# lucidrains/ring-attention-pytorch

Measured on AMD Instinct MI355X. Metric: attn_tflops, higher is better.
Workload: dtype bf16; 1 GPU; model=ring_flash_attn (non-causal, d_head 64), global_batch=1, seq_len=8192, seq_per_gpu=8192, heads=8, kv_heads=8, d_head=64, parallelism=ring1, hipgraph=True

## Files before the change

ring_attention_amd/csrc/attn_fwd.hip:

```cpp

#include <hip/hip_runtime.h>
#include <hip/hip_bf16.h>
#include <cstdint>
#include <cstdlib>

#include "attn_common.h"

namespace ring_attn {

static constexpr int WAVES = 8;
static constexpr int QROWS_WAVE = 32;
static constexpr int QROWS_WG = ROWS_WG;
static_assert(QROWS_WG == WAVES * QROWS_WAVE);
static constexpr int NTHREADS = WAVES * 64;

template <int D>
struct FwdLds {
    static constexpr int KVB = kvblk(D);
    __align__(16) __bf16 k[2][KVB * D];
    __align__(16) __bf16 vt[2][D * KVB];
    unsigned char kmask[2][KVB];
};

template <int D, bool SOFTCLAMP, bool PAIRED>
__global__ __launch_bounds__(NTHREADS, 1) void attn_fwd_kernel(FwdParams p) {
    static_assert(D % 32 == 0);
    constexpr int DBLK = D / 32;
    constexpr int KSTEPS = D / 16;
    constexpr int KVBLK = kvblk(D);
    constexpr int NBLK = KVBLK / 32;

    __shared__ FwdLds<D> lds;

    const int tid = threadIdx.x;
    const int lane = tid & 63;
    const int wid = tid >> 6;
    const int l31 = lane & 31;
    const int lhi = lane >> 5;

    const int bh = blockIdx.y;
    const int b = bh / p.h;
    const int h = bh % p.h;
    const int hk = h % p.hk;

    const int n_pit = PAIRED
        ? (p.paired - 1 - (int)blockIdx.x == (int)blockIdx.x ? 1 : 2) : 1;
    for (int pit = 0; pit < n_pit; ++pit) {
    const int qtile = PAIRED
        ? (pit == 0 ? (int)blockIdx.x : p.paired - 1 - (int)blockIdx.x)
        : (int)blockIdx.x;
    if (PAIRED && pit == 1) {
        __syncthreads();
    }

    if constexpr (PAIRED) {
        auto fwd_body = [&]() {
            const FwdParams P = p;
            #define FWD_EXIT return
            #include "attn_fwd_body.inc"
            #undef FWD_EXIT
        };
        noinline_call(fwd_body);
    } else if constexpr (D == 128) {
        auto fwd_body = [&]() {
            const FwdParams P = p;
            #define FWD_EXIT return
            #include "attn_fwd_body.inc"
            #undef FWD_EXIT
        };
        fwd_body();
    } else {
        const FwdParams& P = p;
        #define FWD_EXIT continue
        #include "attn_fwd_body.inc"
        #undef FWD_EXIT
    }
    }
}

template <int D>
__global__ __launch_bounds__(256) void attn_fwd_merge_kernel(FwdMergeParams p) {
    const long row = (long)blockIdx.x * 256 + threadIdx.x;
    const long total = (long)p.b * p.h * p.nq;
    if (row >= total) return;
    const long bh = row / p.nq;
    const long n = row % p.nq;
    const long b = bh / p.h, h = bh % p.h;

    const long bhn = bh * p.nq + n;
    const long stride_bh = (long)p.b * p.h;

    float m_tot = MASK_VALUE_F;
    if (!p.is_first) m_tot = p.m[bhn];
    for (int s = 0; s < p.splits; ++s)
        m_tot = fmaxf(m_tot, p.m_part[s * stride_bh * p.nq + bhn]);

    float l_tot = 0.f;
    float alpha_prev = 0.f;
    if (!p.is_first) {
        alpha_prev = __expf(p.m[bhn] - m_tot);
        l_tot = p.l[bhn] * alpha_prev;
    }
    float alpha_s[16];
    for (int s = 0; s < p.splits; ++s) {
        alpha_s[s] = __expf(p.m_part[s * stride_bh * p.nq + bhn] - m_tot);
        l_tot += p.l_part[s * stride_bh * p.nq + bhn] * alpha_s[s];
    }

    const long od_base = (bh * D) * p.nq + n;
    if (p.is_last) {
        float l_safe = fmaxf(l_tot, 1e-38f);
        float inv = 1.f / l_safe;
        __bf16* ob = (__bf16*)p.out + ((long)b * p.nq + n) * p.h * D + h * D;
        for (int d = 0; d < D; d += 4) {
            float acc[4];
            #pragma unroll
            for (int e = 0; e < 4; ++e) {
                float v = p.is_first ? 0.f : p.o_acc[od_base + (long)(d + e) * p.nq] * alpha_prev;
                for (int s = 0; s < p.splits; ++s)
                    v += p.o_part[s * stride_bh * D * p.nq + od_base + (long)(d + e) * p.nq]
                         * alpha_s[s];
                acc[e] = v * inv;
            }
            __bf16 four[4] = {(__bf16)acc[0], (__bf16)acc[1], (__bf16)acc[2], (__bf16)acc[3]};
            *(uint2*)(ob + d) = *(uint2*)four;
        }
        p.lse[bhn] = __logf(l_safe) + m_tot;
    } else {
        for (int d = 0; d < D; ++d) {
            float v = p.is_first ? 0.f : p.o_acc[od_base + (long)d * p.nq] * alpha_prev;
            for (int s = 0; s < p.splits; ++s)
                v += p.o_part[s * stride_bh * D * p.nq + od_base + (long)d * p.nq] * alpha_s[s];
            p.o_acc[od_base + (long)d * p.nq] = v;
        }
        p.m[bhn] = m_tot;
        p.l[bhn] = l_tot;
    }
}

void launch_attn_fwd_merge(const FwdMergeParams& p, int head_dim, hipStream_t stream) {
    long total = (long)p.b * p.h * p.nq;
    dim3 grid((total + 255) / 256);
    dim3 block(256);
    if (head_dim == 64) {
        hipLaunchKernelGGL(attn_fwd_merge_kernel<64>, grid, block, 0, stream, p);
    } else if (head_dim == 32) {
        hipLaunchKernelGGL(attn_fwd_merge_kernel<32>, grid, block, 0, stream, p);
    } else {
        hipLaunchKernelGGL(attn_fwd_merge_kernel<128>, grid, block, 0, stream, p);
    }
}

void launch_attn_fwd(const FwdParams& p, int head_dim, hipStream_t stream) {
    static const char* v2env = std::getenv("RING_ATTN_FWD_V2");
    if (v2env && v2env[0] == '1') {
        if (launch_attn_fwd_v2(p, head_dim, stream)) return;
    }
    long qtiles = ceil_div(p.nq, QROWS_WG);
    dim3 grid(p.paired ? (qtiles + 1) / 2 : qtiles, p.b * p.h,
              p.kv_split > 1 ? p.kv_split : 1);
    dim3 block(NTHREADS);
    const bool pr = p.paired > 0;
    if (head_dim == 64) {
        if (p.softclamp) if (pr) hipLaunchKernelGGL((attn_fwd_kernel<64, true, true>), grid, block, 0, stream, p);
        else hipLaunchKernelGGL((attn_fwd_kernel<64, true, false>), grid, block, 0, stream, p);
        else if (pr) hipLaunchKernelGGL((attn_fwd_kernel<64, false, true>), grid, block, 0, stream, p);
        else hipLaunchKernelGGL((attn_fwd_kernel<64, false, false>), grid, block, 0, stream, p);
    } else if (head_dim == 128) {
        if (p.softclamp) if (pr) hipLaunchKernelGGL((attn_fwd_kernel<128, true, true>), grid, block, 0, stream, p);
        else hipLaunchKernelGGL((attn_fwd_kernel<128, true, false>), grid, block, 0, stream, p);
        else if (pr) hipLaunchKernelGGL((attn_fwd_kernel<128, false, true>), grid, block, 0, stream, p);
        else hipLaunchKernelGGL((attn_fwd_kernel<128, false, false>), grid, block, 0, stream, p);
    } else if (head_dim == 32) {
        if (p.softclamp) if (pr) hipLaunchKernelGGL((attn_fwd_kernel<32, true, true>), grid, block, 0, stream, p);
        else hipLaunchKernelGGL((attn_fwd_kernel<32, true, false>), grid, block, 0, stream, p);
        else if (pr) hipLaunchKernelGGL((attn_fwd_kernel<32, false, true>), grid, block, 0, stream, p);
        else hipLaunchKernelGGL((attn_fwd_kernel<32, false, false>), grid, block, 0, stream, p);
    } else {
        __builtin_trap();
    }
}

}
```

ring_attention_amd/csrc/attn_fwd_body.inc:

```
    const long irow0 = (long)qtile * QROWS_WG + wid * QROWS_WAVE;
    const long i = irow0 + l31;
    const bool row_valid = i < P.nq;
    const long i_clamped = row_valid ? i : 0;

    const __bf16* qbase = (const __bf16*)P.q + ((long)b * P.nq + i_clamped) * P.h * D + (long)h * D;
    bf16x8 qf[KSTEPS];
    #pragma unroll
    for (int ks = 0; ks < KSTEPS; ++ks)
        qf[ks] = *(const bf16x8*)(qbase + ks * 16 + lhi * 8);

    float m_run = MASK_VALUE_F;
    float l_run = 0.f;
    f32x16 o_acc[DBLK];
    #pragma unroll
    for (int db = 0; db < DBLK; ++db) o_acc[db] = f32x16{};

    const bool split_mode = P.kv_split > 1;
    const int zsplit = blockIdx.z;
    if (!P.is_first && !split_mode) {
        const float* mrow = P.m + ((long)b * P.h + h) * P.nq;
        const float* lrow = P.l + ((long)b * P.h + h) * P.nq;
        m_run = mrow[i_clamped] * LOG2E;
        l_run = lrow[i_clamped];
        const float* oa = P.o_acc + (((long)b * P.h + h) * D) * P.nq;
        #pragma unroll
        for (int db = 0; db < DBLK; ++db)
            #pragma unroll
            for (int r = 0; r < 16; ++r) {
                int d = db * 32 + (r & 3) + 8 * (r >> 2) + 4 * lhi;
                o_acc[db][r] = oa[(long)d * P.nq + i_clamped];
            }
    }

    const Mask M = mask_of(P);
    const long wg_i_min = (long)qtile * QROWS_WG;
    const long wg_i_max = min((long)(qtile + 1) * QROWS_WG, P.nq) - 1;
    const long wg_q_min = M.qpos(wg_i_min);
    const long wg_q_max = M.qpos(wg_i_max);
    const long qpos_i = M.qpos(i);
    TileRange tr = M.kv_tile_range(wg_i_min, wg_i_max, P.nk, KVBLK);
    if (split_mode) tr = split_share(tr, P.kv_split, zsplit);
    const int t_lo = tr.lo, t_hi = tr.hi;

    constexpr int CH_PER_ROW = D * 2 / 16;
    constexpr int KCHUNKS = KVBLK * CH_PER_ROW;
    constexpr int KREGS = (KCHUNKS + NTHREADS - 1) / NTHREADS;
    constexpr int VPAIRS = (KVBLK / 2) * (D / 8);
    constexpr int VREGS = (VPAIRS + NTHREADS - 1) / NTHREADS;
    const __bf16* kbase = (const __bf16*)P.k + ((long)b * P.nk) * P.hk * D + (long)hk * D;
    const __bf16* vbase = (const __bf16*)P.v + ((long)b * P.nk) * P.hk * D + (long)hk * D;
    const unsigned char* mbase = P.kmask ? (const unsigned char*)P.kmask + (long)b * P.nk : nullptr;

    uint4 kst[KREGS];
    bf16x8 vsta[VREGS], vstb[VREGS];
    unsigned char mst = 1;

    const long kv_row_stride = (long)P.hk * D;
    const long tile_stride = KVBLK * kv_row_stride;
    const __bf16* kptr = kbase + (long)t_lo * tile_stride
        + (tid / CH_PER_ROW) * kv_row_stride + (tid % CH_PER_ROW) * 8;
    const __bf16* vptra = vbase + (long)t_lo * tile_stride
        + ((tid % (KVBLK / 2)) * 2) * kv_row_stride + (tid / (KVBLK / 2)) * 8;
    const __bf16* vptrb = vptra + kv_row_stride;
    long j0_next = (long)t_lo * KVBLK;

    auto load_tile = [&]() {
        const long j0 = j0_next;
        const long jmax = min(j0 + KVBLK, P.nk) - 1;
        const bool full = jmax - j0 == KVBLK - 1;
        #pragma unroll
        for (int r = 0; r < KREGS; ++r) {
            int c = tid + r * NTHREADS;
            if (c < KCHUNKS) {
                const __bf16* src = kptr + (long)(r * (NTHREADS / CH_PER_ROW)) * kv_row_stride;
                kst[r] = (full || (j0 + c / CH_PER_ROW) <= jmax)
                         ? *(const uint4*)src : uint4{0, 0, 0, 0};
            }
        }
        #pragma unroll
        for (int r = 0; r < VREGS; ++r) {
            int c = tid + r * NTHREADS;
            if (c < VPAIRS) {
                const __bf16* sa = vptra + r * (NTHREADS / (KVBLK / 2)) * 8;
                const __bf16* sb = vptrb + r * (NTHREADS / (KVBLK / 2)) * 8;
                long ja = j0 + (c % (KVBLK / 2)) * 2;
                vsta[r] = (full || ja <= jmax) ? *(const bf16x8*)sa : bf16x8{};
                vstb[r] = (full || ja + 1 <= jmax) ? *(const bf16x8*)sb : bf16x8{};
            }
        }
        if (mbase && tid < KVBLK)
            mst = (j0 + tid <= jmax) ? mbase[j0 + tid] : 0;
        kptr += tile_stride;
        vptra += tile_stride;
        vptrb += tile_stride;
        j0_next += KVBLK;
    };

    auto write_tile = [&](int par) {
        #pragma unroll
        for (int r = 0; r < KREGS; ++r) {
            int c = tid + r * NTHREADS;
            if (c < KCHUNKS) {
                int row = c / CH_PER_ROW, ch = c % CH_PER_ROW;
                *(uint4*)(lds.k[par] + row * D + swz<D / 8>(row, ch) * 8) = kst[r];
            }
        }
        #pragma unroll
        for (int r = 0; r < VREGS; ++r) {
            int c = tid + r * NTHREADS;
            if (c < VPAIRS) {
                int jp = kperm_pair(c % (KVBLK / 2));
                int d0 = (c / (KVBLK / 2)) * 8;
                #pragma unroll
                for (int e = 0; e < 8; ++e) {
                    int d = d0 + e;
                    int byte_off = d * KVBLK * 2 + ((jp * 4) ^ ((d & 7) << 4));
                    __bf16 pair[2] = {vsta[r][e], vstb[r][e]};
                    *(uint32_t*)((char*)lds.vt[par] + byte_off) = *(uint32_t*)pair;
                }
            }
        }
        if (mbase && tid < KVBLK) lds.kmask[par][tid] = mst;
    };

    const float scale2 = P.scale * LOG2E;
    if (t_lo < t_hi) {
        load_tile();
        write_tile(t_lo & 1);
        if (P.ablate == 1) write_tile((t_lo & 1) ^ 1);
        if (t_lo + 1 < t_hi && P.ablate != 1) load_tile();
    }

    for (int t = t_lo; t < t_hi; ++t) {
        const int par = t & 1;
        const long j0 = (long)t * KVBLK;
        const long jmax = min(j0 + KVBLK, P.nk) - 1;
        const bool full_tile =
            (jmax - j0 == KVBLK - 1) &&
            M.uncut(wg_q_min, wg_q_max, j0, jmax) &&
            !P.kmask && !P.bias;

        __syncthreads();
        const bool stamp = P.ticks && blockIdx.x == 0 && bh == 0 && tid == 0
                           && blockIdx.z == 0;
        if (stamp) P.ticks[t * 6 + 0] = __builtin_amdgcn_s_memtime();

        f32x16 s[NBLK];
        #pragma unroll
        for (int kb = 0; kb < NBLK; ++kb) s[kb] = f32x16{};
        __builtin_amdgcn_s_setprio(1);
        #pragma unroll
        for (int kb = 0; kb < NBLK; ++kb) {
            int krow = kb * 32 + l31;
            #pragma unroll
            for (int ks = 0; ks < KSTEPS; ++ks) {
                int chunk = ks * 2 + lhi;
                bf16x8 kf = *(const bf16x8*)(lds.k[par] + krow * D + swz<D / 8>(krow, chunk) * 8);
                s[kb] = __builtin_amdgcn_mfma_f32_32x32x16_bf16(kf, qf[ks], s[kb], 0, 0, 0);
            }
        }
        __builtin_amdgcn_s_setprio(0);
        if (stamp) P.ticks[t * 6 + 1] = __builtin_amdgcn_s_memtime();

        if (P.ablate != 1) {
            if (t + 1 < t_hi) write_tile(par ^ 1);
            if (t + 2 < t_hi) load_tile();
        }
        if (stamp) P.ticks[t * 6 + 2] = __builtin_amdgcn_s_memtime();

        if (P.ablate == 2) {
            uint32_t gfrag[4];
            #pragma unroll
            for (int c = 0; c < 4; ++c) {
                union { float f; uint32_t u; } cv; cv.f = s[0][c];
                gfrag[c] = cv.u;
                asm volatile("" :: "v"(gfrag[c]));
            }
            #pragma unroll
            for (int db = 0; db < DBLK; ++db) {
                int drow = db * 32 + l31;
                #pragma unroll
                for (int ks = 0; ks < NBLK * 2; ++ks) {
                    int chunk = ks * 2 + lhi;
                    bf16x8 vf = *(const bf16x8*)(lds.vt[par] + drow * KVBLK + swz<KVBLK / 8>(drow, chunk) * 8);
                    o_acc[db] = __builtin_amdgcn_mfma_f32_32x32x16_bf16(
                        vf, *(const bf16x8*)gfrag, o_acc[db], 0, 0, 0);
                }
            }
            continue;
        }

        float smax = MASK_VALUE_F;
        if (full_tile) {
            if constexpr (!SOFTCLAMP) {
                #pragma unroll
                for (int kb = 0; kb < NBLK; ++kb)
                    #pragma unroll
                    for (int r = 0; r < 16; ++r)
                        smax = fmaxf(smax, s[kb][r]);
                smax *= scale2;
            } else {
                #pragma unroll
                for (int kb = 0; kb < NBLK; ++kb)
                    #pragma unroll
                    for (int r = 0; r < 16; ++r) {
                        float xs = s[kb][r] * (P.scale * __builtin_amdgcn_rcpf(P.softclamp_value));
                        float x = P.softclamp_value * fast_tanhf(xs) * LOG2E;
                        s[kb][r] = x;
                        smax = fmaxf(smax, x);
                    }
            }
        } else {
            #pragma unroll
            for (int kb = 0; kb < NBLK; ++kb)
                #pragma unroll
                for (int r = 0; r < 16; ++r) {
                    float x;
                    if constexpr (SOFTCLAMP) {
                        float xs = s[kb][r] * (P.scale * __builtin_amdgcn_rcpf(P.softclamp_value));
                        x = P.softclamp_value * fast_tanhf(xs) * LOG2E;
                    } else {
                        x = s[kb][r] * scale2;
                    }
                    long j = j0 + kb * 32 + (r & 3) + 8 * (r >> 2) + 4 * lhi;
                    bool ok = j <= jmax;
                    if (P.bias && ok) {
                        const long bi = P.bias_mat
                            ? (((long)b * P.h + h) * P.nq + i_clamped) * P.nk + j
                            : ((long)b * P.h + h) * P.nk + j;
                        x += P.bias[bi] * LOG2E;
                    }
                    ok = M.attends(qpos_i, j, ok);
                    if (P.kmask) ok = ok && lds.kmask[par][j - j0];
                    if (!ok) x = MASK_VALUE_F;
                    s[kb][r] = x;
                    smax = fmaxf(smax, x);
                }
        }
        smax = fmaxf(smax, cross_half(smax));
        if (stamp) P.ticks[t * 6 + 3] = __builtin_amdgcn_s_memtime();

        float m_new = fmaxf(m_run, smax);
        const bool any_growth = !__all(smax <= m_run);
        const float m_exp = fmaxf(m_new, -1.7e38f);
        const float escale = (full_tile && !SOFTCLAMP) ? scale2 : 1.f;
        alignas(16) uint32_t pk[NBLK * 8];
        float partial[NBLK * 8];
        #pragma unroll
        for (int x2 = 0; x2 < NBLK * 8; ++x2) {
            float e0 = __builtin_amdgcn_exp2f(
                __builtin_fmaf(s[x2 >> 3][(2 * x2) & 15], escale, -m_exp));
            float e1 = __builtin_amdgcn_exp2f(
                __builtin_fmaf(s[x2 >> 3][(2 * x2 + 1) & 15], escale, -m_exp));
            partial[x2] = e0 + e1;
            pk[x2] = pack_bf16x2(e0, e1);
        }
        #pragma unroll
        for (int w = NBLK * 4; w >= 1; w >>= 1)
            #pragma unroll
            for (int x2 = 0; x2 < w; ++x2) partial[x2] += partial[x2 + w];
        float rowsum = partial[0];
        rowsum += cross_half(rowsum);
        if (any_growth) {
            float alpha = __builtin_amdgcn_exp2f(m_run - m_new);
            l_run = l_run * alpha + rowsum;
            #pragma unroll
            for (int db = 0; db < DBLK; ++db)
                #pragma unroll
                for (int r = 0; r < 16; ++r) o_acc[db][r] *= alpha;
            m_run = m_new;
        } else {
            l_run += rowsum;
        }


        if (stamp) P.ticks[t * 6 + 4] = __builtin_amdgcn_s_memtime();
        __builtin_amdgcn_s_setprio(1);
        #pragma unroll
        for (int db = 0; db < DBLK; ++db) {
            int drow = db * 32 + l31;
            #pragma unroll
            for (int ks = 0; ks < NBLK * 2; ++ks) {
                int chunk = ks * 2 + lhi;
                bf16x8 vf = *(const bf16x8*)(lds.vt[par] + drow * KVBLK + swz<KVBLK / 8>(drow, chunk) * 8);
                o_acc[db] = __builtin_amdgcn_mfma_f32_32x32x16_bf16(
                    vf, *(const bf16x8*)(pk + 4 * ks), o_acc[db], 0, 0, 0);
            }
        }
        __builtin_amdgcn_s_setprio(0);
        if (stamp) P.ticks[t * 6 + 5] = __builtin_amdgcn_s_memtime();
    }

    if (!row_valid) FWD_EXIT;

    if (split_mode) {
        const long part = (long)zsplit * P.b * P.h;
        float* mrow = P.m + (part + (long)b * P.h + h) * P.nq;
        float* lrow = P.l + (part + (long)b * P.h + h) * P.nq;
        if (lhi == 0) { mrow[i] = m_run * LN2; lrow[i] = l_run; }
        float* oa = P.o_acc + (part + (long)b * P.h + h) * D * P.nq;
        #pragma unroll
        for (int db = 0; db < DBLK; ++db)
            #pragma unroll
            for (int r = 0; r < 16; ++r) {
                int d = db * 32 + (r & 3) + 8 * (r >> 2) + 4 * lhi;
                oa[(long)d * P.nq + i] = o_acc[db][r];
            }
        FWD_EXIT;
    }

    if (P.is_last) {
        float l_safe = fmaxf(l_run, 1e-38f);
        float inv_l = 1.f / l_safe;
        __bf16* ob = (__bf16*)P.out + ((long)b * P.nq + i) * P.h * D + (long)h * D;
        #pragma unroll
        for (int db = 0; db < DBLK; ++db)
            #pragma unroll
            for (int g = 0; g < 4; ++g) {
                __bf16 four[4];
                #pragma unroll
                for (int e = 0; e < 4; ++e)
                    four[e] = (__bf16)(o_acc[db][g * 4 + e] * inv_l);
                int d = db * 32 + 8 * g + 4 * lhi;
                *(uint2*)(ob + d) = *(uint2*)four;
            }
        if (lhi == 0) {
            float* lsep = P.lse + ((long)b * P.h + h) * P.nq;
            lsep[i] = __logf(l_safe) + m_run * LN2;
        }
    } else {
        float* mrow = P.m + ((long)b * P.h + h) * P.nq;
        float* lrow = P.l + ((long)b * P.h + h) * P.nq;
        if (lhi == 0) { mrow[i] = m_run * LN2; lrow[i] = l_run; }
        float* oa = P.o_acc + (((long)b * P.h + h) * D) * P.nq;
        #pragma unroll
        for (int db = 0; db < DBLK; ++db)
            #pragma unroll
            for (int r = 0; r < 16; ++r) {
                int d = db * 32 + (r & 3) + 8 * (r >> 2) + 4 * lhi;
                oa[(long)d * P.nq + i] = o_acc[db][r];
            }
    }
```

Before: 473.9 TFLOP/s.

## Add lean forward kernel variant without mask, bias, tick or ablation paths

Adds a LEAN template parameter to the forward attention kernel. The launcher selects it when there is no key mask, no bias, no timing buffer and no ablation. In that variant the mask, bias, timestamp and ablation code are compiled out. Tail-tile loads become unconditional loads from a valid fallback address, with out-of-range rows zeroed at LDS write time instead of through per-load selects. The o_acc rescale also goes through a mul_f32 helper. The aim is to cut register pressure, branches and select instructions in the hot loop, at the cost of more template instantiations and a slightly different tail-handling path.

```diff
diff --git a/ring_attention_amd/csrc/attn_fwd.hip b/ring_attention_amd/csrc/attn_fwd.hip
--- a/ring_attention_amd/csrc/attn_fwd.hip
+++ b/ring_attention_amd/csrc/attn_fwd.hip
@@ -22,13 +22,29 @@
     unsigned char kmask[2][KVB];
 };
 
-template <int D, bool SOFTCLAMP, bool PAIRED>
+enum BodyForm {
+    BODY_DIRECT,
+    BODY_LAMBDA,
+    BODY_FRAME,
+};
+
+#ifndef FWD_LEAN_FORM
+#define FWD_LEAN_FORM BODY_DIRECT
+#endif
+constexpr BodyForm fwd_body_form(int d, bool paired, bool lean) {
+    if (lean) return (BodyForm)FWD_LEAN_FORM;
+    return paired ? BODY_FRAME : d == 128 ? BODY_LAMBDA : BODY_DIRECT;
+}
+
+template <int D, bool SOFTCLAMP, bool PAIRED, bool LEAN>
 __global__ __launch_bounds__(NTHREADS, 1) void attn_fwd_kernel(FwdParams p) {
     static_assert(D % 32 == 0);
     constexpr int DBLK = D / 32;
     constexpr int KSTEPS = D / 16;
     constexpr int KVBLK = kvblk(D);
     constexpr int NBLK = KVBLK / 32;
+
+    constexpr BodyForm FORM = fwd_body_form(D, PAIRED, LEAN);
 
     __shared__ FwdLds<D> lds;
 
@@ -53,7 +69,7 @@
         __syncthreads();
     }
 
-    if constexpr (PAIRED) {
+    if constexpr (FORM == BODY_FRAME) {
         auto fwd_body = [&]() {
             const FwdParams P = p;
             #define FWD_EXIT return
@@ -61,7 +77,7 @@
             #undef FWD_EXIT
         };
         noinline_call(fwd_body);
-    } else if constexpr (D == 128) {
+    } else if constexpr (FORM == BODY_LAMBDA) {
         auto fwd_body = [&]() {
             const FwdParams P = p;
             #define FWD_EXIT return
@@ -151,6 +167,17 @@
     }
 }
 
+template <int D, bool LEAN>
+static void launch_fwd_d(const FwdParams& p, dim3 grid, dim3 block, hipStream_t stream) {
+    if (p.softclamp) {
+        if (p.paired > 0) hipLaunchKernelGGL((attn_fwd_kernel<D, true, true, LEAN>), grid, block, 0, stream, p);
+        else hipLaunchKernelGGL((attn_fwd_kernel<D, true, false, LEAN>), grid, block, 0, stream, p);
+    } else {
+        if (p.paired > 0) hipLaunchKernelGGL((attn_fwd_kernel<D, false, true, LEAN>), grid, block, 0, stream, p);
+        else hipLaunchKernelGGL((attn_fwd_kernel<D, false, false, LEAN>), grid, block, 0, stream, p);
+    }
+}
+
 void launch_attn_fwd(const FwdParams& p, int head_dim, hipStream_t stream) {
     static const char* v2env = std::getenv("RING_ATTN_FWD_V2");
     if (v2env && v2env[0] == '1') {
@@ -160,22 +187,16 @@
     dim3 grid(p.paired ? (qtiles + 1) / 2 : qtiles, p.b * p.h,
               p.kv_split > 1 ? p.kv_split : 1);
     dim3 block(NTHREADS);
-    const bool pr = p.paired > 0;
+    const bool lean = !p.kmask && !p.bias && !p.ticks && p.ablate == 0;
     if (head_dim == 64) {
-        if (p.softclamp) if (pr) hipLaunchKernelGGL((attn_fwd_kernel<64, true, true>), grid, block, 0, stream, p);
-        else hipLaunchKernelGGL((attn_fwd_kernel<64, true, false>), grid, block, 0, stream, p);
-        else if (pr) hipLaunchKernelGGL((attn_fwd_kernel<64, false, true>), grid, block, 0, stream, p);
-        else hipLaunchKernelGGL((attn_fwd_kernel<64, false, false>), grid, block, 0, stream, p);
+        if (lean) launch_fwd_d<64, true>(p, grid, block, stream);
+        else launch_fwd_d<64, false>(p, grid, block, stream);
     } else if (head_dim == 128) {
-        if (p.softclamp) if (pr) hipLaunchKernelGGL((attn_fwd_kernel<128, true, true>), grid, block, 0, stream, p);
-        else hipLaunchKernelGGL((attn_fwd_kernel<128, true, false>), grid, block, 0, stream, p);
-        else if (pr) hipLaunchKernelGGL((attn_fwd_kernel<128, false, true>), grid, block, 0, stream, p);
-        else hipLaunchKernelGGL((attn_fwd_kernel<128, false, false>), grid, block, 0, stream, p);
+        if (lean) launch_fwd_d<128, true>(p, grid, block, stream);
+        else launch_fwd_d<128, false>(p, grid, block, stream);
     } else if (head_dim == 32) {
-        if (p.softclamp) if (pr) hipLaunchKernelGGL((attn_fwd_kernel<32, true, true>), grid, block, 0, stream, p);
-        else hipLaunchKernelGGL((attn_fwd_kernel<32, true, false>), grid, block, 0, stream, p);
-        else if (pr) hipLaunchKernelGGL((attn_fwd_kernel<32, false, true>), grid, block, 0, stream, p);
-        else hipLaunchKernelGGL((attn_fwd_kernel<32, false, false>), grid, block, 0, stream, p);
+        if (lean) launch_fwd_d<32, true>(p, grid, block, stream);
+        else launch_fwd_d<32, false>(p, grid, block, stream);
     } else {
         __builtin_trap();
     }
diff --git a/ring_attention_amd/csrc/attn_fwd_body.inc b/ring_attention_amd/csrc/attn_fwd_body.inc
--- a/ring_attention_amd/csrc/attn_fwd_body.inc
+++ b/ring_attention_amd/csrc/attn_fwd_body.inc
@@ -1,3 +1,6 @@
+#define FWD_STAMP(n)                                                          \
+    if constexpr (!LEAN)                                                      \
+        if (stamp) P.ticks[t * 6 + (n)] = __builtin_amdgcn_s_memtime()
     const long irow0 = (long)qtile * QROWS_WG + wid * QROWS_WAVE;
     const long i = irow0 + l31;
     const bool row_valid = i < P.nq;
@@ -49,7 +52,9 @@
     constexpr int VREGS = (VPAIRS + NTHREADS - 1) / NTHREADS;
     const __bf16* kbase = (const __bf16*)P.k + ((long)b * P.nk) * P.hk * D + (long)hk * D;
     const __bf16* vbase = (const __bf16*)P.v + ((long)b * P.nk) * P.hk * D + (long)hk * D;
-    const unsigned char* mbase = P.kmask ? (const unsigned char*)P.kmask + (long)b * P.nk : nullptr;
+    const unsigned char* mbase = nullptr;
+    if constexpr (!LEAN)
+        mbase = P.kmask ? (const unsigned char*)P.kmask + (long)b * P.nk : nullptr;
 
     uint4 kst[KREGS];
     bf16x8 vsta[VREGS], vstb[VREGS];
@@ -63,33 +68,59 @@
         + ((tid % (KVBLK / 2)) * 2) * kv_row_stride + (tid / (KVBLK / 2)) * 8;
     const __bf16* vptrb = vptra + kv_row_stride;
     long j0_next = (long)t_lo * KVBLK;
+    long j0_staged = j0_next;
 
     auto load_tile = [&]() {
         const long j0 = j0_next;
         const long jmax = min(j0 + KVBLK, P.nk) - 1;
         const bool full = jmax - j0 == KVBLK - 1;
-        #pragma unroll
-        for (int r = 0; r < KREGS; ++r) {
-            int c = tid + r * NTHREADS;
-            if (c < KCHUNKS) {
-                const __bf16* src = kptr + (long)(r * (NTHREADS / CH_PER_ROW)) * kv_row_stride;
-                kst[r] = (full || (j0 + c / CH_PER_ROW) <= jmax)
-                         ? *(const uint4*)src : uint4{0, 0, 0, 0};
-            }
-        }
-        #pragma unroll
-        for (int r = 0; r < VREGS; ++r) {
-            int c = tid + r * NTHREADS;
-            if (c < VPAIRS) {
-                const __bf16* sa = vptra + r * (NTHREADS / (KVBLK / 2)) * 8;
-                const __bf16* sb = vptrb + r * (NTHREADS / (KVBLK / 2)) * 8;
-                long ja = j0 + (c % (KVBLK / 2)) * 2;
-                vsta[r] = (full || ja <= jmax) ? *(const bf16x8*)sa : bf16x8{};
-                vstb[r] = (full || ja + 1 <= jmax) ? *(const bf16x8*)sb : bf16x8{};
-            }
-        }
-        if (mbase && tid < KVBLK)
-            mst = (j0 + tid <= jmax) ? mbase[j0 + tid] : 0;
+        if constexpr (LEAN) {
+            constexpr int KROW_STEP = NTHREADS / CH_PER_ROW;
+            constexpr int VD_STEP = (NTHREADS / (KVBLK / 2)) * 8;
+            #pragma unroll
+            for (int r = 0; r < KREGS; ++r) {
+                int c = tid + r * NTHREADS;
+                if (c < KCHUNKS) {
+                    const bool ok = full || (j0 + c / CH_PER_ROW) <= jmax;
+                    kst[r] = *(const uint4*)(ok ? kptr + (long)(r * KROW_STEP) * kv_row_stride
+                                                : kbase + (tid % CH_PER_ROW) * 8);
+                }
+            }
+            #pragma unroll
+            for (int r = 0; r < VREGS; ++r) {
+                int c = tid + r * NTHREADS;
+                if (c < VPAIRS) {
+                    const long ja = j0 + (c % (KVBLK / 2)) * 2;
+                    const __bf16* row0 = vbase + (tid / (KVBLK / 2)) * 8 + r * VD_STEP;
+                    vsta[r] = *(const bf16x8*)((full || ja <= jmax) ? vptra + r * VD_STEP : row0);
+                    vstb[r] = *(const bf16x8*)((full || ja + 1 <= jmax) ? vptrb + r * VD_STEP : row0);
+                }
+            }
+            j0_staged = j0;
+        } else {
+            #pragma unroll
+            for (int r = 0; r < KREGS; ++r) {
+                int c = tid + r * NTHREADS;
+                if (c < KCHUNKS) {
+                    const __bf16* src = kptr + (long)(r * (NTHREADS / CH_PER_ROW)) * kv_row_stride;
+                    kst[r] = (full || (j0 + c / CH_PER_ROW) <= jmax)
+                             ? *(const uint4*)src : uint4{0, 0, 0, 0};
+                }
+            }
+            #pragma unroll
+            for (int r = 0; r < VREGS; ++r) {
+                int c = tid + r * NTHREADS;
+                if (c < VPAIRS) {
+                    const __bf16* sa = vptra + r * (NTHREADS / (KVBLK / 2)) * 8;
+                    const __bf16* sb = vptrb + r * (NTHREADS / (KVBLK / 2)) * 8;
+                    long ja = j0 + (c % (KVBLK / 2)) * 2;
+                    vsta[r] = (full || ja <= jmax) ? *(const bf16x8*)sa : bf16x8{};
+                    vstb[r] = (full || ja + 1 <= jmax) ? *(const bf16x8*)sb : bf16x8{};
+                }
+            }
+            if (mbase && tid < KVBLK)
+                mst = (j0 + tid <= jmax) ? mbase[j0 + tid] : 0;
+        }
         kptr += tile_stride;
         vptra += tile_stride;
         vptrb += tile_stride;
@@ -97,6 +128,20 @@
     };
 
     auto write_tile = [&](int par) {
+        if constexpr (LEAN) {
+            const long rows = P.nk - j0_staged;
+            if (rows < KVBLK) {
+                #pragma unroll
+                for (int r = 0; r < KREGS; ++r)
+                    if ((tid + r * NTHREADS) / CH_PER_ROW >= rows) kst[r] = uint4{0, 0, 0, 0};
+                #pragma unroll
+                for (int r = 0; r < VREGS; ++r) {
+                    const int la = ((tid + r * NTHREADS) % (KVBLK / 2)) * 2;
+                    if (la >= rows) vsta[r] = bf16x8{};
+                    if (la + 1 >= rows) vstb[r] = bf16x8{};
+                }
+            }
+        }
         #pragma unroll
         for (int r = 0; r < KREGS; ++r) {
             int c = tid + r * NTHREADS;
@@ -120,30 +165,37 @@
                 }
             }
         }
-        if (mbase && tid < KVBLK) lds.kmask[par][tid] = mst;
+        if constexpr (!LEAN)
+            if (mbase && tid < KVBLK) lds.kmask[par][tid] = mst;
     };
 
     const float scale2 = P.scale * LOG2E;
     if (t_lo < t_hi) {
         load_tile();
         write_tile(t_lo & 1);
-        if (P.ablate == 1) write_tile((t_lo & 1) ^ 1);
-        if (t_lo + 1 < t_hi && P.ablate != 1) load_tile();
+        if constexpr (LEAN) {
+            if (t_lo + 1 < t_hi) load_tile();
+        } else {
+            if (P.ablate == 1) write_tile((t_lo & 1) ^ 1);
+            if (t_lo + 1 < t_hi && P.ablate != 1) load_tile();
+        }
     }
 
     for (int t = t_lo; t < t_hi; ++t) {
         const int par = t & 1;
         const long j0 = (long)t * KVBLK;
         const long jmax = min(j0 + KVBLK, P.nk) - 1;
-        const bool full_tile =
+        bool full_tile =
             (jmax - j0 == KVBLK - 1) &&
-            M.uncut(wg_q_min, wg_q_max, j0, jmax) &&
-            !P.kmask && !P.bias;
+            M.uncut(wg_q_min, wg_q_max, j0, jmax);
+        if constexpr (!LEAN) full_tile = full_tile && !P.kmask && !P.bias;
 
         __syncthreads();
-        const bool stamp = P.ticks && blockIdx.x == 0 && bh == 0 && tid == 0
-                           && blockIdx.z == 0;
-        if (stamp) P.ticks[t * 6 + 0] = __builtin_amdgcn_s_memtime();
+        bool stamp = false;
+        if constexpr (!LEAN)
+            stamp = P.ticks && blockIdx.x == 0 && bh == 0 && tid == 0
+                    && blockIdx.z == 0;
+        FWD_STAMP(0);
 
         f32x16 s[NBLK];
         #pragma unroll
@@ -160,15 +212,17 @@
             }
         }
         __builtin_amdgcn_s_setprio(0);
-        if (stamp) P.ticks[t * 6 + 1] = __builtin_amdgcn_s_memtime();
-
-        if (P.ablate != 1) {
+        FWD_STAMP(1);
+
+        bool restage = true;
+        if constexpr (!LEAN) restage = P.ablate != 1;
+        if (restage) {
             if (t + 1 < t_hi) write_tile(par ^ 1);
             if (t + 2 < t_hi) load_tile();
         }
-        if (stamp) P.ticks[t * 6 + 2] = __builtin_amdgcn_s_memtime();
-
-        if (P.ablate == 2) {
+        FWD_STAMP(2);
+
+        if constexpr (!LEAN) if (P.ablate == 2) {
             uint32_t gfrag[4];
             #pragma unroll
             for (int c = 0; c < 4; ++c) {
@@ -224,21 +278,22 @@
                     }
                     long j = j0 + kb * 32 + (r & 3) + 8 * (r >> 2) + 4 * lhi;
                     bool ok = j <= jmax;
-                    if (P.bias && ok) {
+                    if constexpr (!LEAN) if (P.bias && ok) {
                         const long bi = P.bias_mat
                             ? (((long)b * P.h + h) * P.nq + i_clamped) * P.nk + j
                             : ((long)b * P.h + h) * P.nk + j;
                         x += P.bias[bi] * LOG2E;
                     }
                     ok = M.attends(qpos_i, j, ok);
-                    if (P.kmask) ok = ok && lds.kmask[par][j - j0];
+                    if constexpr (!LEAN)
+                        if (P.kmask) ok = ok && lds.kmask[par][j - j0];
                     if (!ok) x = MASK_VALUE_F;
                     s[kb][r] = x;
                     smax = fmaxf(smax, x);
                 }
         }
         smax = fmaxf(smax, cross_half(smax));
-        if (stamp) P.ticks[t * 6 + 3] = __builtin_amdgcn_s_memtime();
+        FWD_STAMP(3);
 
         float m_new = fmaxf(m_run, smax);
         const bool any_growth = !__all(smax <= m_run);
@@ -267,14 +322,17 @@
             #pragma unroll
             for (int db = 0; db < DBLK; ++db)
                 #pragma unroll
-                for (int r = 0; r < 16; ++r) o_acc[db][r] *= alpha;
+                for (int r = 0; r < 16; ++r) {
+                    if constexpr (LEAN) o_acc[db][r] = mul_f32(o_acc[db][r], alpha);
+                    else o_acc[db][r] *= alpha;
+                }
             m_run = m_new;
         } else {
             l_run += rowsum;
         }
 
 
-        if (stamp) P.ticks[t * 6 + 4] = __builtin_amdgcn_s_memtime();
+        FWD_STAMP(4);
         __builtin_amdgcn_s_setprio(1);
         #pragma unroll
         for (int db = 0; db < DBLK; ++db) {
@@ -288,7 +346,7 @@
             }
         }
         __builtin_amdgcn_s_setprio(0);
-        if (stamp) P.ticks[t * 6 + 5] = __builtin_amdgcn_s_memtime();
+        FWD_STAMP(5);
     }
 
     if (!row_valid) FWD_EXIT;
@@ -341,3 +399,5 @@
                 oa[(long)d * P.nq + i] = o_acc[db][r];
             }
     }
+
+#undef FWD_STAMP
```

After: 484.0 TFLOP/s (median of 6 runs). 1.02x the previous value.
